# Project-MONAI/MONAI

Hardware: NVIDIA H100
Metric: voxels/sec sliding-window inference (higher is better)
Workload: dtype f16

## Files before the change

### monai_b200/_kernels.py

```python
from __future__ import annotations

import ctypes as C
import os
import weakref
from typing import Sequence

import torch

from . import _lib as L


class _Prof:
    on = False
    events: list = []


def profile_start() -> None:
    _Prof.on, _Prof.events = True, []


def profile_stop(by_shape: bool = False) -> dict:
    torch.cuda.synchronize()
    _Prof.on = False
    out: dict = {}
    for name, e0, e1, flops, nbytes in _Prof.events:
        if by_shape:
            name = f"{name} [{flops / 1e9:.2f} GF, {nbytes / 1e6:.1f} MB]"
        d = out.setdefault(name, {"ms": 0.0, "n": 0, "flops": 0.0, "bytes": 0.0})
        d["ms"] += e0.elapsed_time(e1)
        d["n"] += 1
        d["flops"] += flops
        d["bytes"] += nbytes
    _Prof.events = []
    return out


def _call(name: str, *args, flops: float = 0.0, nbytes: float = 0.0) -> None:
    fn = getattr(L.load(), "b200_" + name)
    dev = L.take_stream_device()
    if dev is not None and dev.index is not None and dev.index != torch.cuda.current_device():
        with torch.cuda.device(dev):
            return _call_on(fn, name, args, flops, nbytes)
    return _call_on(fn, name, args, flops, nbytes)


def _call_on(fn, name, args, flops, nbytes) -> None:
    if _Prof.on:
        e0, e1 = torch.cuda.Event(enable_timing=True), torch.cuda.Event(enable_timing=True)
        e0.record()
        rc = fn(*args)
        e1.record()
        _Prof.events.append((name, e0, e1, flops, nbytes))
    else:
        rc = fn(*args)
    L.check(rc, name)


_F32_CACHE: dict = {}


def _f32c(t: torch.Tensor | None) -> torch.Tensor | None:
    if t is None:
        return None
    src = t
    t = t.detach()
    if t.dtype == torch.float32 and t.is_contiguous():
        return t
    key = (id(src), tuple(t.shape), t.dtype, t.device)
    hit = _F32_CACHE.get(key)
    if hit is not None and hit[0]() is src and hit[1] == src._version and hit[2] == src.data_ptr():
        return hit[3]
    val = t.to(torch.float32).contiguous()
    try:
        ref = weakref.ref(src, lambda _r, k=key: _F32_CACHE.pop(k, None))
    except TypeError:
        return val
    _F32_CACHE[key] = (ref, src._version, src.data_ptr(), val)
    return val


def _ws(nbytes: int, device) -> torch.Tensor | None:
    if nbytes < 0:
        raise ValueError("monai_b200: workspace query failed for this shape")
    return torch.empty(max(int(nbytes), 16), device=device, dtype=torch.uint8)


# ... 548 lines not shown


def patch_merge_ln_nc8(x: NC8, gamma: torch.Tensor, beta: torch.Tensor, eps: float = 1e-5, v2: bool = False) -> NC8:
    sp2 = tuple((s + 1) // 2 for s in x.sp)
    out = NC8(x.N, 8 * x.C, sp2, x.buf.device)
    g, b = _f32c(gamma), _f32c(beta)
    _call("patch_merge_ln_nc8", L.ptr(x.buf), x.N, x.C, x.sp[0], x.sp[1], x.sp[2], L.ptr(g), L.ptr(b), float(eps), int(v2), L.ptr(out.buf), L.stream_ptr(x.buf.device))
    return out


def window_attention_nc8(qkv: NC8, Cc: int, heads: int, nW: int, n: int, scale: float, table: torch.Tensor, window: Sequence[int],
                         region: torch.Tensor | None) -> NC8:
    out = NC8(qkv.N, Cc, qkv.sp, qkv.buf.device)
    tab = _f32c(table)
    _call("window_attention_nc8", L.ptr(qkv.buf), qkv.N, Cc, heads, nW, n, float(scale), L.ptr(tab), int(window[0]), int(window[1]), int(window[2]),
          L.ptr(region), L.ptr(out.buf), L.stream_ptr(qkv.buf.device), flops=4.0 * qkv.N * nW * heads * n * n * 16,
          nbytes=float(qkv.N * 4 * Cc * nW * n * 2))
    return out


def window_attention_tc_plan(region, nW: int, n: int):
    import numpy as np

    if region is None:
        types = np.zeros(nW, dtype=np.int64)
        reps = None
        ntypes = 1
    else:
        region = np.asarray(region).reshape(nW, n)
        canon = np.empty_like(region)
        for w in range(nW):
            _, first, inv = np.unique(region[w], return_index=True, return_inverse=True)
            order = np.argsort(np.argsort(first))
            canon[w] = order[inv]
        uniq, types = np.unique(canon, axis=0, return_inverse=True)
        types = types.reshape(-1)
        ntypes = int(uniq.shape[0])
        reps = uniq.astype(np.int32)
    sched = np.zeros(16 + nW, dtype=np.int32)
    if ntypes <= 8:
        pos = 0
        for t in range(ntypes):
            ids = np.nonzero(types == t)[0]
            sched[t], sched[8 + t] = len(ids), pos
            sched[16 + pos: 16 + pos + len(ids)] = ids
            pos += len(ids)
    return sched, reps, ntypes


def window_attention_tc_pack_bias(table: torch.Tensor, heads: int, n: int, window: Sequence[int], region_types: torch.Tensor | None, ntypes: int) -> torch.Tensor:
    tab = _f32c(table)
    nbytes = L.load().b200_window_attention_tc_bias_bytes(heads, n, ntypes)
    if nbytes < 0:
        raise ValueError(f"window_attention_tc: unsupported shape (n={n}, mask types={ntypes})")
    packed = torch.empty(nbytes // 2, device=tab.device, dtype=torch.float16)
    _call("window_attention_tc_pack_bias", L.ptr(tab), heads, n, int(window[0]), int(window[1]), int(window[2]), L.ptr(region_types), ntypes,
          L.ptr(packed), L.stream_ptr(tab.device))
    return packed


def window_attention_tc(qkv: NC8, Cc: int, heads: int, nW: int, n: int, packed_bias: torch.Tensor, sched: torch.Tensor, ntypes: int) -> NC8:
    out = NC8(qkv.N, Cc, qkv.sp, qkv.buf.device)
    n_pad = (n + 31) // 32 * 32
    _call("window_attention_tc", L.ptr(qkv.buf), qkv.N, Cc, heads, nW, n, L.ptr(packed_bias), L.ptr(sched), ntypes, L.ptr(out.buf),
          L.stream_ptr(qkv.buf.device), flops=4.0 * qkv.N * nW * heads * n * n * 16, nbytes=float(qkv.N * 4 * Cc * nW * n * 2))
    return out


def mhsa_tc(qkv: NC8, C_: int, heads: int) -> NC8:
    if qkv.C != 3 * C_:
        raise ValueError(f"mhsa_tc: qkv has {qkv.C} channels, expected 3 * {C_}")
    out = NC8(qkv.N, C_, qkv.sp, qkv.buf.device)
    S = qkv.S
    try:
        _call("mhsa_tc", L.ptr(qkv.buf), qkv.N, C_, heads, S, L.ptr(out.buf), L.stream_ptr(qkv.buf.device),
              flops=4.0 * qkv.N * heads * S * S * 64, nbytes=float(qkv.N * 4 * C_ * S * 2))
    except RuntimeError as e:
        if C_ != 64 * heads:
            raise ValueError(str(e)) from None
        raise
    return out


ATTN_TC = not bool(os.environ.get("B200_ATTN_HMMA"))
LOG2E = 1.4426950408889634


def conv_cin1_nc8(x: torch.Tensor, weight: torch.Tensor, bias: torch.Tensor | None, k: int, stride: int, pad: int,
                  out: NC8 | None = None, out_coff: int = 0, want_stats: bool = False) -> tuple[NC8, torch.Tensor | None]:
    L.require_cuda(x)
    x = x.contiguous()
    N, _, D, H, W = x.shape
    Cout = weight.shape[0]
    sp = tuple((s + 2 * pad - k) // stride + 1 for s in (D, H, W))
    if out is None:
        out = NC8(N, Cout, sp, x.device)
    w32 = _f32c(weight)
    b32 = _f32c(bias)
    stats = torch.empty((N * Cout, 2), device=x.device, dtype=torch.float32) if want_stats else None
    tc = (k, stride, pad) in ((3, 1, 1), (2, 2, 0)) and Cout in (16, 32, 48, 64, 96, 128)
    name = "conv_cin1_tc" if tc else "conv_cin1_nc8"
    ws = None
    if want_stats:
        ws = _ws(getattr(L.load(), f"b200_{name}_workspace_bytes")(N, D, H, W, Cout, k, stride, pad), x.device)
    _call(name, L.ptr(x), L.dt(x), N, D, H, W, L.ptr(w32), L.ptr(b32), Cout, k, stride, pad, L.ptr(out.buf), out.C, out_coff, L.ptr(stats), L.ptr(ws),
          L.stream_ptr(x.device), flops=2.0 * N * sp[0] * sp[1] * sp[2] * Cout * k**3, nbytes=_nb(x) + float(N * sp[0] * sp[1] * sp[2] * Cout * 2))
    return out, stats


def head_conv_nc8(x: NC8, weight: torch.Tensor, bias: torch.Tensor | None, out_dtype: torch.dtype = torch.float16) -> torch.Tensor:
    Cout = weight.shape[0]
    w32 = _f32c(weight)
    b32 = _f32c(bias)
    y = torch.empty((x.N, Cout, *x.sp), device=x.buf.device, dtype=out_dtype)
    _call("head_conv_nc8", L.ptr(x.buf), x.N, x.C, x.S, L.ptr(w32), L.ptr(b32), Cout, L.ptr(y), L.dt(y), L.stream_ptr(x.buf.device))
    return y


def head_conv_norm_nc8(x: NC8, stats: torch.Tensor, res: NC8 | None, res_coff: int, res_stats: torch.Tensor | None, slope: float, eps: float,
                       weight: torch.Tensor, bias: torch.Tensor | None, out_dtype: torch.dtype = torch.float16) -> torch.Tensor:
    Cout = weight.shape[0]
    w32 = _f32c(weight)
    b32 = _f32c(bias)
    y = torch.empty((x.N, Cout, *x.sp), device=x.buf.device, dtype=out_dtype)
    _call("head_conv_norm_nc8", L.ptr(x.buf), x.N, x.C, x.S, L.ptr(stats), float(eps), L.ptr(res.buf) if res is not None else None,
          res.C if res is not None else 0, res_coff, L.ptr(res_stats), float(slope), L.ptr(w32), L.ptr(b32), Cout, L.ptr(y), L.dt(y),
          L.stream_ptr(x.buf.device), nbytes=float(x.N * x.S * (x.C * (4 if res is not None else 2) + Cout * y.element_size())))
    return y


def _cg_desc(x_sp, N, Cin, Cout, k, stride, pad, transposed, output_padding, in_ctot, in_coff, out_ctot, out_coff, out_layout, out_dtype):
    sp_out = conv_out_shape(x_sp, (k,) * 3, (stride,) * 3, (pad,) * 3, transposed, (output_padding,) * 3)
    return L.ConvGatherDesc(N, Cin, Cout, x_sp[0], x_sp[1], x_sp[2], sp_out[0], sp_out[1], sp_out[2], k, stride, pad, int(transposed),
                            in_ctot, in_coff, out_ctot, out_coff, out_layout, out_dtype), sp_out


def conv_gather_tc_pack_weight(weight: torch.Tensor, k: int, stride: int, pad: int, transposed: bool) -> torch.Tensor:
    L.require_cuda(weight)
    Cin, Cout = (weight.shape[0], weight.shape[1]) if transposed else (weight.shape[1], weight.shape[0])
    d, _ = _cg_desc((8, 8, 8), 1, Cin, Cout, k, stride, pad, transposed, stride - 1 if transposed else 0, Cin, 0, (Cout + 7) // 8 * 8, 0, 1, L.DT_F16)
    nbytes = L.load().b200_conv_gather_tc_weight_bytes(C.byref(d))
    if nbytes < 0:
        raise ValueError(f"conv_gather_tc needs Cin % 16 == 0, kernel <= 3, stride <= 2 (got Cin={Cin}, k={k}, stride={stride})")
    w32 = weight.detach().float().contiguous()
    packed = torch.empty(nbytes // 2, device=weight.device, dtype=torch.float16)
    _call("conv_gather_tc_pack_weight", C.byref(d), L.ptr(w32), L.ptr(packed), L.stream_ptr(weight.device))
    return packed


def conv_gather_tc(
    x: NC8, packed_w: torch.Tensor, Cin: int, Cout: int, k: int, stride: int, pad: int, transposed: bool = False, output_padding: int = 0,
    in_coff: int = 0, bias: torch.Tensor | None = None, out: "NC8 | torch.Tensor | None" = None, out_coff: int = 0,
    ncdhw_dtype: torch.dtype | None = None, want_stats: bool = False,
):
    layout = 0 if ncdhw_dtype is None else 1
    d, sp_out = _cg_desc(x.sp, x.N, Cin, Cout, k, stride, pad, transposed, output_padding, x.C, in_coff,
                         (out.C if isinstance(out, NC8) else (Cout + 7) // 8 * 8), out_coff, layout, L.dt(ncdhw_dtype) if layout else L.DT_F16)
    if out is None:
        out = NC8(x.N, Cout, sp_out, x.buf.device) if layout == 0 else torch.empty((x.N, Cout, *sp_out), device=x.buf.device, dtype=ncdhw_dtype)
        d.out_ctot = out.C if layout == 0 else d.out_ctot
    stats = torch.empty((x.N * Cout, 2), device=x.buf.device, dtype=torch.float32) if want_stats else None
    b32 = _f32c(bias)
    taps = k**3 if not transposed else (k**3) / (stride**3)
    ws = _ws(L.load().b200_conv_gather_tc_workspace_bytes(C.byref(d)), x.buf.device) if want_stats else None
    _call("conv_gather_tc", C.byref(d), L.ptr(x.buf), L.ptr(packed_w), L.ptr(b32), L.ptr(out.buf if layout == 0 else out), L.ptr(stats), L.ptr(ws),
          L.stream_ptr(x.buf.device), flops=2.0 * x.N * sp_out[0] * sp_out[1] * sp_out[2] * Cin * Cout * taps,
          nbytes=float(x.N * (x.S * Cin + sp_out[0] * sp_out[1] * sp_out[2] * Cout) * 2) + _nb(packed_w))
# ... 10 lines not shown
```

### monai_b200/csrc/attn_tc.cu

```cuda
#include "common.cuh"
#include "tc90.cuh"
#include "../../include/monai_b200.h"

namespace b200 {

constexpr int kAtNPadMax = 352;
constexpr int kAtKChunk = kAtNPadMax * 16;
constexpr int kAtBiasBytes = 16 * kAtNPadMax * 16;
constexpr int kAtIdBytes = 16 * 2048;
constexpr int kAtQBytes = 2 * 2048, kAtKBytes = 2 * kAtKChunk, kAtVBytes = 2 * kAtKChunk;
constexpr int kAtSmem = kAtBiasBytes + kAtIdBytes + 2 * (kAtQBytes + kAtKBytes + kAtVBytes) + 2 * 2 * tc::kStageFloats * 4 + 256 + 128;
constexpr float kAtPadBias = -30000.f;

struct AttnTcParams {
  const __half* qkv; __half* out; const __half* bias; const int32_t* sched;
  int N, C8, heads, nW, n, n_pad, nrt, ntypes;
};

struct AttnTile { int ty, h, rt, b, w; };

__device__ __forceinline__ AttnTile attn_decode(const AttnTcParams& p, long long f) {
  const int32_t* cnt = p.sched;
  const int32_t* start = p.sched + 8;
  const int32_t* win = p.sched + 16;
  AttnTile t;
  t.ty = 0;
  const long long hr_n = (long long)p.heads * p.nrt;
  for (;;) {
    const long long blk = (long long)cnt[t.ty] * p.N * hr_n;
    if (f < blk || t.ty + 1 >= p.ntypes) break;
    f -= blk; ++t.ty;
  }
  const int c = cnt[t.ty];
  const long long per = (long long)c * p.N;
  const int hr = (int)(f / per);
  const int l2 = (int)(f % per);
  t.h = hr / p.nrt; t.rt = hr % p.nrt;
  t.b = l2 / c;
  t.w = win[start[t.ty] + l2 % c];
  return t;
}

__device__ __forceinline__ float ex2(float x) {
  float y;
  asm("ex2.approx.ftz.f32 %0, %1;" : "=f"(y) : "f"(x));
  return y;
}

__device__ __forceinline__ uint32_t exp2_pack(float a, float b, float m, float& sum) {
  const __half2 h = __floats2half2_rn(ex2(a - m), ex2(b - m));
  const float2 r = __half22float2(h);
  sum += r.x + r.y;
  return *reinterpret_cast<const uint32_t*>(&h);
}

constexpr int kAtThreads = 384;

template <int NPAD>
__global__ void __launch_bounds__(kAtThreads, 1) window_attention_tc_kernel(AttnTcParams p) {
  extern __shared__ uint8_t smem_raw[];
  uint8_t* smem = tc::align_smem128(smem_raw);
  uint8_t* s_bias = smem;
  uint8_t* s_id = s_bias + kAtBiasBytes;
  uint8_t* s_q = s_id + kAtIdBytes;
  uint8_t* s_k = s_q + 2 * kAtQBytes;
  uint8_t* s_v = s_k + 2 * kAtKBytes;
  float* s_stage = reinterpret_cast<float*>(s_v + 2 * kAtVBytes);
  uint64_t* bars = reinterpret_cast<uint64_t*>(s_stage + 2 * 2 * tc::kStageFloats);
  uint64_t* qk_full = bars + 0;
  uint64_t* qk_empty = bars + 2;
  uint64_t* v_full = bars + 4;
  uint64_t* v_empty = bars + 6;

  const int warp = __shfl_sync(0xffffffffu, threadIdx.x >> 5, 0), lane = threadIdx.x & 31;
  constexpr int n_pad = NPAD;
  const int n = p.n;
  const long long T = (long long)p.nW * n;
  const long long total = (long long)p.N * p.nW * p.heads * p.nrt;
  const long long lo = total * blockIdx.x / gridDim.x, hi = total * (blockIdx.x + 1) / gridDim.x;

  if (threadIdx.x == 0) {
    for (int i = 0; i < 2; ++i) {
      tc::mbar_init(&qk_full[i], 1); tc::mbar_init(&qk_empty[i], 2); tc::mbar_init(&v_full[i], 1); tc::mbar_init(&v_empty[i], 2);
    }
    tc::fence_barrier_init();
  }
  {
    const uint4 z = make_uint4(0, 0, 0, 0);
    uint4* zq = reinterpret_cast<uint4*>(s_id);
    const int nz = (kAtIdBytes + 2 * kAtQBytes + 2 * kAtKBytes + 2 * kAtVBytes) / 16;
    for (int i = threadIdx.x; i < nz; i += blockDim.x) zq[i] = z;
  }
  __syncthreads();
  {
    __half* id = reinterpret_cast<__half*>(s_id);
    for (int r = threadIdx.x; r < 128; r += blockDim.x) id[((r >> 3) * 128 + r) * 8 + (r & 7)] = __float2half_rn(1.f);
  }
  tc::fence_proxy_async();
  __syncthreads();

  if (warp == 0) {
    if (lane == 0) {
      int last_combo = -1;
      int it = 0;
      for (long long f = lo; f < hi; ++f, ++it) {
        const AttnTile t = attn_decode(p, f);
        const int combo = (t.ty * p.heads + t.h) * p.nrt + t.rt;
        const int rows = min(128, n - t.rt * 128);
        const int b = it & 1;
        const uint32_t use = (uint32_t)((it >> 1) & 1);
        tc::mbar_wait(&qk_empty[b], use ^ 1u);
        uint32_t bias_bytes = 0u;
        if (combo != last_combo) {
          if (it > 0) tc::mbar_wait(&qk_empty[b ^ 1], (uint32_t)(((it - 1) >> 1) & 1));
          bias_bytes = (uint32_t)(16 * n_pad * 16);
        }
        tc::mbar_arrive_expect_tx(&qk_full[b], bias_bytes + 2u * rows * 16u + 2u * n * 16u);
        if (bias_bytes) tc::bulk_load(s_bias, p.bias + (long long)combo * (16 * n_pad * 8), bias_bytes, &qk_full[b]);
        last_combo = combo;
        const __half* base = p.qkv + (long long)t.b * (3 * p.C8) * T * 8;
        const long long row0 = (long long)t.w * n;
        for (int c = 0; c < 2; ++c) {
          tc::bulk_load(s_q + b * kAtQBytes + c * 2048, base + ((long long)(2 * t.h + c) * T + row0 + t.rt * 128) * 8, rows * 16, &qk_full[b]);
          tc::bulk_load(s_k + b * kAtKBytes + c * kAtKChunk, base + ((long long)(p.C8 + 2 * t.h + c) * T + row0) * 8, n * 16, &qk_full[b]);
        }
        tc::mbar_wait(&v_empty[b], use ^ 1u);
        tc::mbar_arrive_expect_tx(&v_full[b], 2u * n * 16u);
        for (int c = 0; c < 2; ++c)
          tc::bulk_load(s_v + b * kAtVBytes + c * kAtKChunk, base + ((long long)(2 * p.C8 + 2 * t.h + c) * T + row0) * 8, n * 16, &v_full[b]);
      }
    }
    __syncwarp();
  } else if (warp >= 4) {
    const int g = (warp >> 2) - 1, wid = warp & 3;
    const uint32_t q_a = tc::smem_u32(s_q), k_a = tc::smem_u32(s_k), v_a = tc::smem_u32(s_v), b_a = tc::smem_u32(s_bias),
                   i_a = tc::smem_u32(s_id);
    float* stage = s_stage + g * 2 * tc::kStageFloats;
    int sl = 0;
    int it = 0;
    for (long long f = lo; f < hi; ++f, ++it) {
      const int b = it & 1;
      const uint32_t use = (uint32_t)((it >> 1) & 1);
      float o[8];
#pragma unroll
      for (int j = 0; j < 8; ++j) o[j] = 0.f;
      float m0 = -INFINITY, m1 = -INFINITY, l0 = 0.f, l1 = 0.f;
      tc::mbar_wait(&qk_full[b], use);
      tc::mbar_wait(&v_full[b], use);
      const uint64_t qd = tc::make_desc_kmajor_noswz(q_a + b * kAtQBytes + g * 1024, 2048, 128);
#pragma unroll 1
      for (int kb = 0; kb < n_pad / 32; ++kb) {
        float sc[16];
        tc::wg_fence();
        tc::Mma<32>::ss<0>(sc, qd, tc::make_desc_kmajor_noswz(k_a + b * kAtKBytes + kb * 32 * 16, kAtKChunk, 128), 0u);
#pragma unroll
        for (int s4 = 0; s4 < 4; ++s4) {
          const int ks = 4 * g + s4;
          const uint64_t id_d = tc::make_desc_kmajor_noswz(i_a + ks * 4096 + g * 1024, 2048, 128);
          const uint64_t bd = tc::make_desc_kmajor_noswz(b_a + (2 * ks) * n_pad * 16 + kb * 32 * 16, n_pad * 16, 128);
          tc::Mma<32>::ss<0>(sc, id_d, bd, 1u);
        }
        tc::wg_commit();
        tc::wg_wait<0>();
        tc::wg_fence_acc<16>(sc);
        float x0 = sc[0], x1 = sc[2];
#pragma unroll
        for (int i = 0; i < 4; ++i) {
          x0 = fmaxf(x0, fmaxf(sc[4 * i], sc[4 * i + 1]));
          x1 = fmaxf(x1, fmaxf(sc[4 * i + 2], sc[4 * i + 3]));
        }
        x0 = fmaxf(x0, __shfl_xor_sync(0xffffffffu, x0, 1)); x0 = fmaxf(x0, __shfl_xor_sync(0xffffffffu, x0, 2));
        x1 = fmaxf(x1, __shfl_xor_sync(0xffffffffu, x1, 1)); x1 = fmaxf(x1, __shfl_xor_sync(0xffffffffu, x1, 2));
        const float n0 = fmaxf(m0, x0), n1 = fmaxf(m1, x1);
        const float a0 = ex2(m0 - n0), a1 = ex2(m1 - n1);
        m0 = n0; m1 = n1;
        l0 *= a0; l1 *= a1;
#pragma unroll
        for (int i = 0; i < 2; ++i) { o[4 * i] *= a0; o[4 * i + 1] *= a0; o[4 * i + 2] *= a1; o[4 * i + 3] *= a1; }
        uint32_t pa[2][4];
#pragma unroll
        for (int kk = 0; kk < 2; ++kk) {
          pa[kk][0] = exp2_pack(sc[8 * kk + 0], sc[8 * kk + 1], m0, l0);
          pa[kk][1] = exp2_pack(sc[8 * kk + 2], sc[8 * kk + 3], m1, l1);
          pa[kk][2] = exp2_pack(sc[8 * kk + 4], sc[8 * kk + 5], m0, l0);
          pa[kk][3] = exp2_pack(sc[8 * kk + 6], sc[8 * kk + 7], m1, l1);
        }
        tc::wg_fence();
#pragma unroll
        for (int kk = 0; kk < 2; ++kk) {
          const uint64_t vd = tc::make_desc_kmajor_noswz(v_a + b * kAtVBytes + (2 * kb + kk) * 256, 128, kAtKChunk);
          tc::Mma<16>::rs<1>(o, pa[kk], vd, 1u);
        }
        tc::wg_commit();
        tc::wg_wait<0>();
        tc::wg_fence_acc<8>(o);
#pragma unroll
        for (int kk = 0; kk < 2; ++kk)
#pragma unroll
          for (int j = 0; j < 4; ++j) asm volatile("" : "+r"(pa[kk][j])::"memory");
      }
      if (wid == 0 && lane == 0) { tc::mbar_arrive(&qk_empty[b]); tc::mbar_arrive(&v_empty[b]); }
      l0 += __shfl_xor_sync(0xffffffffu, l0, 1); l0 += __shfl_xor_sync(0xffffffffu, l0, 2);
      l1 += __shfl_xor_sync(0xffffffffu, l1, 1); l1 += __shfl_xor_sync(0xffffffffu, l1, 2);
      const float i0 = 1.f / l0, i1 = 1.f / l1;
#pragma unroll
      for (int i = 0; i < 2; ++i) { o[4 * i] *= i0; o[4 * i + 1] *= i0; o[4 * i + 2] *= i1; o[4 * i + 3] *= i1; }
      float* buf = stage + (sl & 1) * tc::kStageFloats;
      ++sl;
      tc::wg_stage16<0>(o, buf, wid, lane);
      tc::wg_bar(8 + g);
      float v[8];
      tc::wg_read8(buf, wid, lane, v);
      const AttnTile t = attn_decode(p, f);
      const int r = t.rt * 128 + 64 * g + 32 * (wid & 1) + lane;
      if (r < n) {
        const int dt = wid >> 1;
        __half* ob = p.out + (long long)t.b * p.C8 * T * 8 + ((long long)t.w * n + r) * 8;
        uint4 hv;
        __half2* hp = reinterpret_cast<__half2*>(&hv);
#pragma unroll
        for (int j = 0; j < 4; ++j) hp[j] = __floats2half2_rn(v[2 * j], v[2 * j + 1]);
        *reinterpret_cast<uint4*>(ob + (long long)(2 * t.h + dt) * T * 8) = hv;
      }
    }
  }
}

__global__ void attn_bias_pack_kernel(const float* __restrict__ table, const int32_t* __restrict__ region, __half* __restrict__ out,
                                      int heads, int n, int n_pad, int nrt, int ntypes, int ws0, int ws1, int ws2) {
  const long long total = (long long)ntypes * heads * nrt * 16 * n_pad * 8;
  const int s1 = 2 * ws2 - 1, s0 = (2 * ws1 - 1) * s1;
  const int lin_c = (ws0 - 1) * s0 + (ws1 - 1) * s1 + (ws2 - 1);
  constexpr float kLog2e = 1.4426950408889634f;
  for (long long i = (long long)blockIdx.x * blockDim.x + threadIdx.x; i < total; i += (long long)gridDim.x * blockDim.x) {
    long long r = i;
    const int e = (int)(r % 8); r /= 8;
    const int j = (int)(r % n_pad); r /= n_pad;
    const int c = (int)(r % 16); r /= 16;
    const int rt = (int)(r % nrt); r /= nrt;
    const int h = (int)(r % heads); r /= heads;
    const int ty = (int)r;
    const int ig = rt * 128 + c * 8 + e;
    float v;
    if (j >= n) v = kAtPadBias;
    else if (ig >= n) v = 0.f;
    else {
      const int li = (ig / (ws1 * ws2)) * s0 + ((ig / ws2) % ws1) * s1 + ig % ws2;
      const int lj = (j / (ws1 * ws2)) * s0 + ((j / ws2) % ws1) * s1 + j % ws2;
      v = table[(long long)(li - lj + lin_c) * heads + h] * kLog2e;
      if (region && region[(long long)ty * n + ig] != region[(long long)ty * n + j]) v += -100.f * kLog2e;
    }
    out[i] = __float2half_rn(v);
  }
}

}

using namespace b200;

static bool attn_tc_shape_ok(int heads, int n, int ntypes) {
  return heads > 0 && n > 0 && n <= kAtNPadMax && ntypes >= 1 && ntypes <= 8;
}

extern "C" long long b200_window_attention_tc_bias_bytes(int heads, int n, int ntypes) {
  if (!attn_tc_shape_ok(heads, n, ntypes) || n > kAtNPadMax) return -1;
  const int n_pad = (n + 31) / 32 * 32, nrt = (n + 127) / 128;
  return (long long)ntypes * heads * nrt * 16 * n_pad * 16;
}

extern "C" int b200_window_attention_tc_pack_bias(const float* table, int heads, int n, int ws0, int ws1, int ws2,
                                                  const int32_t* region_types, int ntypes, void* packed, void* stream) {
  B200_REQUIRE(table && packed, "window_attention_tc_pack_bias: null pointer");
  B200_REQUIRE(attn_tc_shape_ok(heads, n, ntypes) && n <= kAtNPadMax, "window_attention_tc: unsupported shape (n = %d, types = %d)", n, ntypes);
  B200_REQUIRE(ws0 > 0 && ws1 > 0 && ws2 > 0 && n <= ws0 * ws1 * ws2, "window_attention_tc: window of %d tokens exceeds the module window", n);
  B200_REQUIRE(ntypes == 1 || region_types, "window_attention_tc_pack_bias: several mask types need their region rows");
  const int n_pad = (n + 31) / 32 * 32, nrt = (n + 127) / 128;
  const long long total = (long long)ntypes * heads * nrt * 16 * n_pad * 8;
  const int blocks = (int)std::min<long long>((total + 255) / 256, 8192);
  attn_bias_pack_kernel<<<blocks, 256, 0, (cudaStream_t)stream>>>(table, region_types, (__half*)packed, heads, n, n_pad, nrt, ntypes, ws0, ws1, ws2);
  B200_LAUNCH_CHECK("attn_bias_pack_kernel");
  return B200_OK;
}

extern "C" int b200_window_attention_tc(const void* qkv, int N, int C, int heads, int nW, int n, const void* packed_bias,
                                        const int32_t* sched, int ntypes, void* out, void* stream) {
  B200_REQUIRE(qkv && out && packed_bias && sched, "window_attention_tc: null pointer");
  B200_REQUIRE(N > 0 && nW > 0, "window_attention_tc: empty problem");
  B200_REQUIRE(C == heads * 16, "window_attention_tc: head_dim must be 16 (C = %d, heads = %d)", C, heads);
  B200_REQUIRE(attn_tc_shape_ok(heads, n, ntypes) && n <= kAtNPadMax, "window_attention_tc: unsupported shape (n = %d, types = %d)", n, ntypes);
  AttnTcParams p;
  p.qkv = (const __half*)qkv; p.out = (__half*)out; p.bias = (const __half*)packed_bias; p.sched = sched;
  p.N = N; p.C8 = C / 8; p.heads = heads; p.nW = nW; p.n = n; p.n_pad = (n + 31) / 32 * 32; p.nrt = (n + 127) / 128; p.ntypes = ntypes;
  const long long total = (long long)N * nW * heads * p.nrt;
  dim3 grid((unsigned)std::min<long long>(total, num_sms()));
  void (*kern)(AttnTcParams) = nullptr;
  switch (p.n_pad) {
#define B200_ATTN_CASE(NP) case NP: kern = window_attention_tc_kernel<NP>; break;
    B200_ATTN_CASE(32) B200_ATTN_CASE(64) B200_ATTN_CASE(96) B200_ATTN_CASE(128) B200_ATTN_CASE(160) B200_ATTN_CASE(192)
    B200_ATTN_CASE(224) B200_ATTN_CASE(256) B200_ATTN_CASE(288) B200_ATTN_CASE(320) B200_ATTN_CASE(352)
#undef B200_ATTN_CASE
  }
  B200_REQUIRE(kern != nullptr, "window_attention_tc: no kernel for %d padded keys", p.n_pad);
  B200_CUDA(cudaFuncSetAttribute(kern, cudaFuncAttributeMaxDynamicSharedMemorySize, kAtSmem));
  kern<<<grid, kAtThreads, kAtSmem, (cudaStream_t)stream>>>(p);
  B200_LAUNCH_CHECK("window_attention_tc_kernel");
  return B200_OK;
}
```

### monai_b200/networks/nets/swin_unetr.py

```python
from __future__ import annotations

import itertools
from collections.abc import Sequence

import numpy as np
import torch
import torch.nn as nn

from ... import _kernels as K
from ... import _lib as L
from .._graph import GraphedForward
from ._tc_blocks import TcBlocks, _Cache
from ..blocks.acti_norm import norm_act_from_modules
from ..blocks.convolutions import Convolution, run_conv_module

__all__ = ["SwinUNETR", "PatchMerging", "PatchMergingV2", "window_plan"]


def _rep(v, n):
    return tuple(v) if isinstance(v, (list, tuple)) else (v,) * n


class PatchEmbed(nn.Module):

# ... 209 lines not shown
    ) -> None:
        super().__init__()
        if spatial_dims not in (2, 3):
            raise ValueError("spatial dimension should be 2 or 3.")
        for name, v in (("dropout rate", drop_rate), ("attention dropout rate", attn_drop_rate), ("drop path rate", dropout_path_rate)):
            if not (0 <= v <= 1):
                raise ValueError(f"{name} should be between 0 and 1.")
        if feature_size % 12 != 0:
            raise ValueError("feature_size should be divisible by 12.")
        if spatial_dims != 3:
            raise NotImplementedError("monai_b200 SwinUNETR implements spatial_dims=3")
        head_dims = [(feature_size * 2**i) // h for i, h in enumerate(num_heads)]
        if any((feature_size * 2**i) % h for i, h in enumerate(num_heads)) or any(d not in (8, 16, 24, 32, 48, 64) for d in head_dims):
            raise NotImplementedError(f"monai_b200 window attention supports head dimensions 8, 16, 24, 32, 48, 64 (got {head_dims})")
        self._tc_ok = feature_size % 48 == 0 and all(d == 16 for d in head_dims)
        self.fp32_faithful = False
        nn_name = norm_name if isinstance(norm_name, str) else norm_name[0]
        if str(nn_name).lower() != "instance" or (not isinstance(norm_name, str) and norm_name[1].get("affine")):
            raise NotImplementedError("monai_b200 SwinUNETR implements norm_name='instance' (non-affine)")
        if patch_size != 2:
            raise NotImplementedError("monai_b200 SwinUNETR implements patch_size=2")
        self.patch_size = patch_size
        self.normalize = normalize
        self.feature_size = feature_size
        self.out_channels = out_channels
        self.in_channels = in_channels
        if in_channels < 1:
            raise ValueError("in_channels must be positive")
        self.use_v2 = use_v2
        ws = _rep(window_size, 3)
        self.swinViT = SwinTransformer(in_channels, feature_size, ws, _rep(patch_size, 3), depths, num_heads, mlp_ratio, qkv_bias,
                                       norm_layer, patch_norm, downsample, use_v2)
        fs = feature_size
        self.encoder1 = UnetrBasicBlock(in_channels, fs)
        self.encoder2 = UnetrBasicBlock(fs, fs)
        self.encoder3 = UnetrBasicBlock(2 * fs, 2 * fs)
        self.encoder4 = UnetrBasicBlock(4 * fs, 4 * fs)
        self.encoder10 = UnetrBasicBlock(16 * fs, 16 * fs)
        self.decoder5 = UnetrUpBlock(16 * fs, 8 * fs)
        self.decoder4 = UnetrUpBlock(8 * fs, 4 * fs)
        self.decoder3 = UnetrUpBlock(4 * fs, 2 * fs)
        self.decoder2 = UnetrUpBlock(2 * fs, fs)
        self.decoder1 = UnetrUpBlock(fs, fs)
        self.out = UnetOutBlock(fs, out_channels)
        self._cache = _Cache()
        self._graph_init()

    def _check_input_size(self, spatial_shape):
        img_size = np.array(spatial_shape)
        remainder = (img_size % np.power(self.patch_size, 5)) > 0
        if remainder.any():
            wrong_dims = (np.where(remainder)[0] + 2).tolist()
            raise ValueError(
                f"spatial dimensions {wrong_dims} of input image (spatial shape: {spatial_shape})"
                f" must be divisible by {self.patch_size}**5."
            )

    def _plan(self, dims, ws, ss, dev):
        def build():
            src, region, nW, n = window_plan(dims, ws, ss)
            sched, reps, ntypes = K.window_attention_tc_plan(region, nW, n)
            tc = None
            if ntypes <= 8 and n <= 352:
                tc = (torch.from_numpy(sched).to(dev), None if reps is None else torch.from_numpy(reps).contiguous().to(dev), ntypes)
            return (torch.from_numpy(src).to(dev), None if region is None else torch.from_numpy(region).to(dev), nW, n, tc)

        return self._cache.get(("plan", tuple(dims), tuple(ws), tuple(ss), dev), [], build)

    def _attn_bias(self, attn: WindowAttention, key, n: int, tc):
        _, reps, ntypes = tc
        return self._cache.get(("attnb", key, n, ntypes, attn.relative_position_bias_table.device), [attn.relative_position_bias_table],
                               lambda: K.window_attention_tc_pack_bias(attn.relative_position_bias_table, attn.num_heads, n, attn.window_size, reps, ntypes))

    def _swin_stage(self, cur: K.NC8, layer: BasicLayer, key: str, pre: UnetrBasicBlock | None = None) -> K.NC8:
        dims, C = cur.sp, cur.C
        dev = cur.buf.device
        if pre is not None:
            cur = self._res_block(cur, C, 0, pre.layer, key + ".c")
        for bi, blk in enumerate(layer.blocks):
            ws, ss = _get_window_size(dims, blk.window_size, blk.shift_size)
            src, region, nW, n, tc = self._plan(dims, ws, ss, dev)
            bkey = f"{key}.b{bi}"
            xw = K.layernorm_nc8(cur, blk.norm1.weight, blk.norm1.bias, blk.norm1.eps, src=src, out_sp=(1, nW, n))
            if K.ATTN_TC and tc is not None:
                wq, bq = self._wqkv_scaled(blk.attn.qkv.weight, blk.attn.qkv.bias, C, blk.attn.scale, bkey)
                qkv, _ = K.gemm_tc(xw, wq, C, 3 * C, bias=bq)
                att = K.window_attention_tc(qkv, C, blk.num_heads, nW, n, self._attn_bias(blk.attn, (bkey, tuple(dims), tuple(ws), tuple(ss)), n, tc), tc[0], tc[2])
            else:
                qkv, _ = K.gemm_tc(xw, self._wlin(blk.attn.qkv.weight, bkey + ".qkv"), C, 3 * C, bias=blk.attn.qkv.bias)
                att = K.window_attention_nc8(qkv, C, blk.num_heads, nW, n, blk.attn.scale, blk.attn.relative_position_bias_table, blk.attn.window_size,
                                             region if any(s > 0 for s in ss) else None)
            x1, _ = K.gemm_tc(att, self._wlin(blk.attn.proj.weight, bkey + ".proj"), C, C, bias=blk.attn.proj.bias, res=cur, row_map=src, out_sp=dims, mode=1)
            hid = blk.mlp.linear1.out_features
            w1, w2 = self._wlin(blk.mlp.linear1.weight, bkey + ".fc1"), self._wlin(blk.mlp.linear2.weight, bkey + ".fc2")
            if K.mlp_fused_supported(C, hid):
                cur = K.mlp_fused_tc(x1, w1, blk.mlp.linear1.bias, w2, blk.mlp.linear2.bias, hid, blk.norm2.weight, blk.norm2.bias, blk.norm2.eps)
            else:
                y = K.layernorm_nc8(x1, blk.norm2.weight, blk.norm2.bias, blk.norm2.eps)
                h, _ = K.gemm_tc(y, w1, C, hid, bias=blk.mlp.linear1.bias, act=L.ACT_GELU)
                cur, _ = K.gemm_tc(h, w2, hid, C, bias=blk.mlp.linear2.bias, res=x1)
        if layer.downsample is not None:
            ds = layer.downsample
            m = K.patch_merge_ln_nc8(cur, ds.norm.weight, ds.norm.bias, ds.norm.eps, v2=ds.v2)
            cur, _ = K.gemm_tc(m, self._wlin(ds.reduction.weight, key + ".red"), 8 * C, 2 * C)
        return cur

    def _proj_out(self, t: K.NC8, out: K.NC8 | None = None, out_coff: int = 0) -> K.NC8:
        if not self.normalize:
            if out is None:
                return t
            return K.norm_act_nc8(t, t.C, None, out=out, out_coff=out_coff)
        if out is None:
            return K.layernorm_nc8(t, None, None, 1e-5)
        tmp = K.layernorm_nc8(t, None, None, 1e-5)
        return K.norm_act_nc8(tmp, t.C, None, out=out, out_coff=out_coff)

    def forward(self, x_in: torch.Tensor) -> torch.Tensor:
        if not x_in.is_cuda:
            raise RuntimeError("monai_b200.SwinUNETR runs on CUDA tensors only (there is no CPU fallback)")
        self._check_input_size(x_in.shape[2:])
        if x_in.shape[1] != self.in_channels:
            raise ValueError(f"expected {self.in_channels} input channel(s), got {x_in.shape[1]}")
        if x_in.dtype not in (torch.float16, torch.float32):
            raise TypeError(f"SwinUNETR takes float16/float32 inputs, got {x_in.dtype}")
        if not self._tc_ok or self.fp32_faithful:
            return self._forward_direct(x_in)
        if x_in.dtype == torch.float32 and not getattr(self, "_warned_fp32", False):
            import warnings

            warnings.warn("monai_b200.SwinUNETR computes with fp16 activation storage (fp32 accumulation); float32 inputs are converted. "
                          "Expect ~1e-2 relative agreement with an fp32 reference, not 1e-3 (set net.fp32_faithful = True for the fp32 path).")
            self._warned_fp32 = True
        if self._graph_ok():
            return self._forward_graphed(x_in, self._forward_impl)
        return self._forward_impl(x_in)

    def _plan_direct(self, dims, ws, ss, dev):
        key = ("plan_direct", tuple(dims), tuple(ws), tuple(ss), dev)
        hit = self._cache.store.get(key)
        if hit is None:
            src, region, nW, n = window_plan(dims, ws, ss)
            inv = np.full(int(np.prod(dims)), -1, dtype=np.int32)
            rows = np.nonzero(src >= 0)[0]
            inv[src[rows]] = rows.astype(np.int32)
            hit = (torch.from_numpy(src).to(dev), None if region is None else torch.from_numpy(np.ascontiguousarray(region)).to(dev),
                   torch.from_numpy(inv).to(dev), nW, n)
            self._cache.store[key] = hit
        return hit

    def _dense_bias(self, attn: WindowAttention, n: int, key):
        def build():
            idx = attn.relative_position_index[:n, :n].reshape(-1)
            return attn.relative_position_bias_table.detach().float()[idx].reshape(n, n, -1).permute(2, 0, 1).contiguous()

        return self._cache.get(("dense_bias", key, n, attn.relative_position_bias_table.device), [attn.relative_position_bias_table], build)

    def _merge_params(self, ds, C: int, key):
        def build():
            order = list(itertools.product(range(2), range(2), range(2))) if ds.v2 else \
                [(0, 0, 0), (1, 0, 0), (0, 1, 0), (0, 0, 1), (1, 1, 0), (1, 0, 1), (0, 1, 1), (1, 1, 1)]
            ref_of_pat = np.empty(8 * C, dtype=np.int64)
            for k, (a, b, e) in enumerate(order):
                for c in range(C):
                    ref_of_pat[c * 8 + a * 4 + b * 2 + e] = k * C + c
            idx = torch.from_numpy(ref_of_pat).to(ds.norm.weight.device)
            return (ds.norm.weight.detach().float()[idx].contiguous(), ds.norm.bias.detach().float()[idx].contiguous(),
                    ds.reduction.weight.detach().float()[:, idx].contiguous())
# ... 149 lines not shown
```

Measured before the change: 55.56 million.

## Restructure window attention kernel: three consumer warpgroups, bias preloaded into accumulators, pipelined QK/PV

Rewrites the tensor-core window attention kernel to use three consumer warpgroups covering 192 query rows, up from two covering 128. The relative position bias is now repacked into accumulator-fragment layout and loaded straight into the score registers, replacing the extra identity-matrix MMAs that added it before. The QK^T MMA for the next 64-key chunk is issued while softmax and the PV MMA of the current chunk run. Register budgets are rebalanced with setmaxnreg, and the schedule groups tiles so bias reloads happen less often. The trade-offs are higher register pressure and more complex synchronisation, and the environment switch that selected the older fallback path is removed.

```diff
diff --git a/monai_b200/_kernels.py b/monai_b200/_kernels.py
--- a/monai_b200/_kernels.py
+++ b/monai_b200/_kernels.py
@@ -1,7 +1,6 @@
 from __future__ import annotations
 
 import ctypes as C
-import os
 import weakref
 from typing import Sequence
 
@@ -716,7 +715,6 @@
     return out
 
 
-ATTN_TC = not bool(os.environ.get("B200_ATTN_HMMA"))
 LOG2E = 1.4426950408889634
 
 
diff --git a/monai_b200/csrc/attn_tc.cu b/monai_b200/csrc/attn_tc.cu
--- a/monai_b200/csrc/attn_tc.cu
+++ b/monai_b200/csrc/attn_tc.cu
@@ -5,12 +5,15 @@
 namespace b200 {
 
 constexpr int kAtNPadMax = 352;
+constexpr int kAtWG = 3;
+constexpr int kAtRows = 64 * kAtWG;
+constexpr int kAtCT = 128 * kAtWG;
 constexpr int kAtKChunk = kAtNPadMax * 16;
-constexpr int kAtBiasBytes = 16 * kAtNPadMax * 16;
-constexpr int kAtIdBytes = 16 * 2048;
-constexpr int kAtQBytes = 2 * 2048, kAtKBytes = 2 * kAtKChunk, kAtVBytes = 2 * kAtKChunk;
-constexpr int kAtSmem = kAtBiasBytes + kAtIdBytes + 2 * (kAtQBytes + kAtKBytes + kAtVBytes) + 2 * 2 * tc::kStageFloats * 4 + 256 + 128;
+constexpr int kAtBiasBytes = kAtNPadMax * kAtCT;
+constexpr int kAtQBytes = 2 * kAtRows * 16, kAtKBytes = 2 * kAtKChunk, kAtVBytes = 2 * kAtKChunk;
+constexpr int kAtSmem = kAtBiasBytes + 2 * (kAtQBytes + kAtKBytes + kAtVBytes) + kAtWG * 2 * tc::kStageFloats * 4 + 256 + 128;
 constexpr float kAtPadBias = -30000.f;
+constexpr int kAtGroup = 8;
 
 struct AttnTcParams {
   const __half* qkv; __half* out; const __half* bias; const int32_t* sched;
@@ -32,10 +35,23 @@
     f -= blk; ++t.ty;
   }
   const int c = cnt[t.ty];
-  const long long per = (long long)c * p.N;
-  const int hr = (int)(f / per);
-  const int l2 = (int)(f % per);
-  t.h = hr / p.nrt; t.rt = hr % p.nrt;
+  const int per = c * p.N;
+  const long long per_h = (long long)per * p.nrt;
+  t.h = (int)(f / per_h);
+  int r = (int)(f % per_h);
+  const int full = per / kAtGroup * kAtGroup;
+  int l2;
+  if (r < full * p.nrt) {
+    const int grp = r / (kAtGroup * p.nrt);
+    r %= kAtGroup * p.nrt;
+    t.rt = r / kAtGroup;
+    l2 = grp * kAtGroup + r % kAtGroup;
+  } else {
+    r -= full * p.nrt;
+    const int rem = per - full;
+    t.rt = r / rem;
+    l2 = full + r % rem;
+  }
   t.b = l2 / c;
   t.w = win[start[t.ty] + l2 % c];
   return t;
@@ -54,19 +70,28 @@
   return *reinterpret_cast<const uint32_t*>(&h);
 }
 
-constexpr int kAtThreads = 384;
+__device__ __forceinline__ void bias_to_acc(const uint8_t* src, float* d) {
+  const uint4 v = *reinterpret_cast<const uint4*>(src);
+  const __half2* h = reinterpret_cast<const __half2*>(&v);
+#pragma unroll
+  for (int j = 0; j < 4; ++j) {
+    const float2 f = __half22float2(h[j]);
+    d[2 * j] = f.x; d[2 * j + 1] = f.y;
+  }
+}
+
+constexpr int kAtThreads = 128 * (kAtWG + 1);
 
 template <int NPAD>
 __global__ void __launch_bounds__(kAtThreads, 1) window_attention_tc_kernel(AttnTcParams p) {
   extern __shared__ uint8_t smem_raw[];
   uint8_t* smem = tc::align_smem128(smem_raw);
   uint8_t* s_bias = smem;
-  uint8_t* s_id = s_bias + kAtBiasBytes;
-  uint8_t* s_q = s_id + kAtIdBytes;
+  uint8_t* s_q = s_bias + kAtBiasBytes;
   uint8_t* s_k = s_q + 2 * kAtQBytes;
   uint8_t* s_v = s_k + 2 * kAtKBytes;
   float* s_stage = reinterpret_cast<float*>(s_v + 2 * kAtVBytes);
-  uint64_t* bars = reinterpret_cast<uint64_t*>(s_stage + 2 * 2 * tc::kStageFloats);
+  uint64_t* bars = reinterpret_cast<uint64_t*>(s_stage + kAtWG * 2 * tc::kStageFloats);
   uint64_t* qk_full = bars + 0;
   uint64_t* qk_empty = bars + 2;
   uint64_t* v_full = bars + 4;
@@ -74,6 +99,8 @@
 
   const int warp = __shfl_sync(0xffffffffu, threadIdx.x >> 5, 0), lane = threadIdx.x & 31;
   constexpr int n_pad = NPAD;
+  constexpr int NB = NPAD / 32;
+  constexpr int NC = (NB + 1) / 2;
   const int n = p.n;
   const long long T = (long long)p.nW * n;
   const long long total = (long long)p.N * p.nW * p.heads * p.nrt;
@@ -81,47 +108,43 @@
 
   if (threadIdx.x == 0) {
     for (int i = 0; i < 2; ++i) {
-      tc::mbar_init(&qk_full[i], 1); tc::mbar_init(&qk_empty[i], 2); tc::mbar_init(&v_full[i], 1); tc::mbar_init(&v_empty[i], 2);
+      tc::mbar_init(&qk_full[i], 1); tc::mbar_init(&qk_empty[i], kAtWG); tc::mbar_init(&v_full[i], 1); tc::mbar_init(&v_empty[i], kAtWG);
     }
     tc::fence_barrier_init();
   }
   {
     const uint4 z = make_uint4(0, 0, 0, 0);
-    uint4* zq = reinterpret_cast<uint4*>(s_id);
-    const int nz = (kAtIdBytes + 2 * kAtQBytes + 2 * kAtKBytes + 2 * kAtVBytes) / 16;
+    uint4* zq = reinterpret_cast<uint4*>(s_q);
+    const int nz = (2 * kAtQBytes + 2 * kAtKBytes + 2 * kAtVBytes) / 16;
     for (int i = threadIdx.x; i < nz; i += blockDim.x) zq[i] = z;
-  }
-  __syncthreads();
-  {
-    __half* id = reinterpret_cast<__half*>(s_id);
-    for (int r = threadIdx.x; r < 128; r += blockDim.x) id[((r >> 3) * 128 + r) * 8 + (r & 7)] = __float2half_rn(1.f);
   }
   tc::fence_proxy_async();
   __syncthreads();
 
-  if (warp == 0) {
-    if (lane == 0) {
+  if (warp < 4) {
+    asm volatile("setmaxnreg.dec.sync.aligned.u32 56;\n" ::: "memory");
+    if (warp == 0 && lane == 0) {
       int last_combo = -1;
       int it = 0;
       for (long long f = lo; f < hi; ++f, ++it) {
         const AttnTile t = attn_decode(p, f);
         const int combo = (t.ty * p.heads + t.h) * p.nrt + t.rt;
-        const int rows = min(128, n - t.rt * 128);
+        const int rows = min(kAtRows, n - t.rt * kAtRows);
         const int b = it & 1;
         const uint32_t use = (uint32_t)((it >> 1) & 1);
         tc::mbar_wait(&qk_empty[b], use ^ 1u);
         uint32_t bias_bytes = 0u;
         if (combo != last_combo) {
           if (it > 0) tc::mbar_wait(&qk_empty[b ^ 1], (uint32_t)(((it - 1) >> 1) & 1));
-          bias_bytes = (uint32_t)(16 * n_pad * 16);
+          bias_bytes = (uint32_t)(n_pad * kAtCT);
         }
         tc::mbar_arrive_expect_tx(&qk_full[b], bias_bytes + 2u * rows * 16u + 2u * n * 16u);
-        if (bias_bytes) tc::bulk_load(s_bias, p.bias + (long long)combo * (16 * n_pad * 8), bias_bytes, &qk_full[b]);
+        if (bias_bytes) tc::bulk_load(s_bias, p.bias + (long long)combo * (n_pad * kAtCT / 2), bias_bytes, &qk_full[b]);
         last_combo = combo;
         const __half* base = p.qkv + (long long)t.b * (3 * p.C8) * T * 8;
         const long long row0 = (long long)t.w * n;
         for (int c = 0; c < 2; ++c) {
-          tc::bulk_load(s_q + b * kAtQBytes + c * 2048, base + ((long long)(2 * t.h + c) * T + row0 + t.rt * 128) * 8, rows * 16, &qk_full[b]);
+          tc::bulk_load(s_q + b * kAtQBytes + c * kAtRows * 16, base + ((long long)(2 * t.h + c) * T + row0 + t.rt * kAtRows) * 8, rows * 16, &qk_full[b]);
           tc::bulk_load(s_k + b * kAtKBytes + c * kAtKChunk, base + ((long long)(p.C8 + 2 * t.h + c) * T + row0) * 8, n * 16, &qk_full[b]);
         }
         tc::mbar_wait(&v_empty[b], use ^ 1u);
@@ -130,79 +153,116 @@
           tc::bulk_load(s_v + b * kAtVBytes + c * kAtKChunk, base + ((long long)(2 * p.C8 + 2 * t.h + c) * T + row0) * 8, n * 16, &v_full[b]);
       }
     }
-    __syncwarp();
-  } else if (warp >= 4) {
+  } else {
+    asm volatile("setmaxnreg.inc.sync.aligned.u32 152;\n" ::: "memory");
     const int g = (warp >> 2) - 1, wid = warp & 3;
-    const uint32_t q_a = tc::smem_u32(s_q), k_a = tc::smem_u32(s_k), v_a = tc::smem_u32(s_v), b_a = tc::smem_u32(s_bias),
-                   i_a = tc::smem_u32(s_id);
+    const int ct = threadIdx.x - 128;
+    const uint32_t q_a = tc::smem_u32(s_q), k_a = tc::smem_u32(s_k), v_a = tc::smem_u32(s_v);
     float* stage = s_stage + g * 2 * tc::kStageFloats;
     int sl = 0;
     int it = 0;
     for (long long f = lo; f < hi; ++f, ++it) {
       const int b = it & 1;
       const uint32_t use = (uint32_t)((it >> 1) & 1);
+      const AttnTile t = attn_decode(p, f);
+      const bool dead = t.rt * kAtRows + 64 * g + 16 * wid >= n;
       float o[8];
 #pragma unroll
       for (int j = 0; j < 8; ++j) o[j] = 0.f;
       float m0 = -INFINITY, m1 = -INFINITY, l0 = 0.f, l1 = 0.f;
+      float s[2][32];
+      uint32_t pa[2][4][4];
       tc::mbar_wait(&qk_full[b], use);
       tc::mbar_wait(&v_full[b], use);
-      const uint64_t qd = tc::make_desc_kmajor_noswz(q_a + b * kAtQBytes + g * 1024, 2048, 128);
-#pragma unroll 1
-      for (int kb = 0; kb < n_pad / 32; ++kb) {
-        float sc[16];
+      if (t.rt * kAtRows + 64 * g >= n) {
+        if (wid == 0 && lane == 0) { tc::mbar_arrive(&qk_empty[b]); tc::mbar_arrive(&v_empty[b]); }
+        continue;
+      }
+      const uint64_t qd = tc::make_desc_kmajor_noswz(q_a + b * kAtQBytes + g * 1024, kAtRows * 16, 128);
+
+      auto issue_s = [&](auto cc) {
+        constexpr int c = decltype(cc)::value;
+        constexpr int nb = (2 * c + 1 < NB) ? 2 : 1;
+        float* sc = s[c & 1];
+#pragma unroll
+        for (int k2 = 0; k2 < nb; ++k2)
+#pragma unroll
+          for (int hh = 0; hh < 2; ++hh) bias_to_acc(s_bias + ((2 * c + k2) * 2 + hh) * (kAtCT * 16) + ct * 16, sc + 16 * k2 + 8 * hh);
         tc::wg_fence();
-        tc::Mma<32>::ss<0>(sc, qd, tc::make_desc_kmajor_noswz(k_a + b * kAtKBytes + kb * 32 * 16, kAtKChunk, 128), 0u);
-#pragma unroll
-        for (int s4 = 0; s4 < 4; ++s4) {
-          const int ks = 4 * g + s4;
-          const uint64_t id_d = tc::make_desc_kmajor_noswz(i_a + ks * 4096 + g * 1024, 2048, 128);
-          const uint64_t bd = tc::make_desc_kmajor_noswz(b_a + (2 * ks) * n_pad * 16 + kb * 32 * 16, n_pad * 16, 128);
-          tc::Mma<32>::ss<0>(sc, id_d, bd, 1u);
-        }
+        const uint64_t kd = tc::make_desc_kmajor_noswz(k_a + b * kAtKBytes + c * 64 * 16, kAtKChunk, 128);
+        if constexpr (nb == 2) tc::Mma<64>::ss<0>(sc, qd, kd, 1u);
+        else tc::Mma<32>::ss<0>(sc, qd, kd, 1u);
         tc::wg_commit();
-        tc::wg_wait<0>();
-        tc::wg_fence_acc<16>(sc);
-        float x0 = sc[0], x1 = sc[2];
-#pragma unroll
-        for (int i = 0; i < 4; ++i) {
-          x0 = fmaxf(x0, fmaxf(sc[4 * i], sc[4 * i + 1]));
-          x1 = fmaxf(x1, fmaxf(sc[4 * i + 2], sc[4 * i + 3]));
-        }
-        x0 = fmaxf(x0, __shfl_xor_sync(0xffffffffu, x0, 1)); x0 = fmaxf(x0, __shfl_xor_sync(0xffffffffu, x0, 2));
-        x1 = fmaxf(x1, __shfl_xor_sync(0xffffffffu, x1, 1)); x1 = fmaxf(x1, __shfl_xor_sync(0xffffffffu, x1, 2));
-        const float n0 = fmaxf(m0, x0), n1 = fmaxf(m1, x1);
-        const float a0 = ex2(m0 - n0), a1 = ex2(m1 - n1);
-        m0 = n0; m1 = n1;
-        l0 *= a0; l1 *= a1;
+      };
+
+      issue_s(std::integral_constant<int, 0>{});
+      tc::static_for<0, NC>([&](auto cc) {
+        constexpr int c = decltype(cc)::value;
+        constexpr int nb = (2 * c + 1 < NB) ? 2 : 1;
+        constexpr int nv = 16 * nb;
+        if constexpr (c + 1 < NC) {
+          issue_s(std::integral_constant<int, c + 1>{});
+          if constexpr (c == 0) tc::wg_wait<1>(); else tc::wg_wait<2>();
+        } else {
+          if constexpr (c == 0) tc::wg_wait<0>(); else tc::wg_wait<1>();
+        }
+        float* sc = s[c & 1];
+        tc::wg_fence_acc<nv>(sc);
+        float a0 = 1.f, a1 = 1.f, ps0 = 0.f, ps1 = 0.f;
+        if (!dead) {
+          float x0 = sc[0], x1 = sc[2];
+#pragma unroll
+          for (int i = 0; i < nv / 4; ++i) {
+            x0 = fmaxf(x0, fmaxf(sc[4 * i], sc[4 * i + 1]));
+            x1 = fmaxf(x1, fmaxf(sc[4 * i + 2], sc[4 * i + 3]));
+          }
+          x0 = fmaxf(x0, __shfl_xor_sync(0xffffffffu, x0, 1)); x0 = fmaxf(x0, __shfl_xor_sync(0xffffffffu, x0, 2));
+          x1 = fmaxf(x1, __shfl_xor_sync(0xffffffffu, x1, 1)); x1 = fmaxf(x1, __shfl_xor_sync(0xffffffffu, x1, 2));
+          const float n0 = fmaxf(m0, x0), n1 = fmaxf(m1, x1);
+          a0 = ex2(m0 - n0); a1 = ex2(m1 - n1);
+          m0 = n0; m1 = n1;
+#pragma unroll
+          for (int kk = 0; kk < 2 * nb; ++kk) {
+            pa[c & 1][kk][0] = exp2_pack(sc[8 * kk + 0], sc[8 * kk + 1], m0, ps0);
+            pa[c & 1][kk][1] = exp2_pack(sc[8 * kk + 2], sc[8 * kk + 3], m1, ps1);
+            pa[c & 1][kk][2] = exp2_pack(sc[8 * kk + 4], sc[8 * kk + 5], m0, ps0);
+            pa[c & 1][kk][3] = exp2_pack(sc[8 * kk + 6], sc[8 * kk + 7], m1, ps1);
+          }
+        } else {
+#pragma unroll
+          for (int kk = 0; kk < 2 * nb; ++kk)
+#pragma unroll
+            for (int j = 0; j < 4; ++j) pa[c & 1][kk][j] = 0u;
+        }
+        if constexpr (c > 0) {
+          if constexpr (c + 1 < NC) tc::wg_wait<1>(); else tc::wg_wait<0>();
+          tc::wg_fence_acc<8>(o);
+#pragma unroll
+          for (int kk = 0; kk < 4; ++kk)
+#pragma unroll
+            for (int j = 0; j < 4; ++j) asm volatile("" : "+r"(pa[(c - 1) & 1][kk][j])::"memory");
+        }
+        l0 = l0 * a0 + ps0; l1 = l1 * a1 + ps1;
 #pragma unroll
         for (int i = 0; i < 2; ++i) { o[4 * i] *= a0; o[4 * i + 1] *= a0; o[4 * i + 2] *= a1; o[4 * i + 3] *= a1; }
-        uint32_t pa[2][4];
-#pragma unroll
-        for (int kk = 0; kk < 2; ++kk) {
-          pa[kk][0] = exp2_pack(sc[8 * kk + 0], sc[8 * kk + 1], m0, l0);
-          pa[kk][1] = exp2_pack(sc[8 * kk + 2], sc[8 * kk + 3], m1, l1);
-          pa[kk][2] = exp2_pack(sc[8 * kk + 4], sc[8 * kk + 5], m0, l0);
-          pa[kk][3] = exp2_pack(sc[8 * kk + 6], sc[8 * kk + 7], m1, l1);
-        }
         tc::wg_fence();
 #pragma unroll
-        for (int kk = 0; kk < 2; ++kk) {
-          const uint64_t vd = tc::make_desc_kmajor_noswz(v_a + b * kAtVBytes + (2 * kb + kk) * 256, 128, kAtKChunk);
-          tc::Mma<16>::rs<1>(o, pa[kk], vd, 1u);
+        for (int kk = 0; kk < 2 * nb; ++kk) {
+          const uint64_t vd = tc::make_desc_kmajor_noswz(v_a + b * kAtVBytes + (4 * c + kk) * 256, 128, kAtKChunk);
+          tc::Mma<16>::rs<1>(o, pa[c & 1][kk], vd, 1u);
         }
         tc::wg_commit();
-        tc::wg_wait<0>();
-        tc::wg_fence_acc<8>(o);
-#pragma unroll
-        for (int kk = 0; kk < 2; ++kk)
-#pragma unroll
-          for (int j = 0; j < 4; ++j) asm volatile("" : "+r"(pa[kk][j])::"memory");
-      }
+      });
+      tc::wg_wait<0>();
+      tc::wg_fence_acc<8>(o);
+#pragma unroll
+      for (int kk = 0; kk < 4; ++kk)
+#pragma unroll
+        for (int j = 0; j < 4; ++j) asm volatile("" : "+r"(pa[(NC - 1) & 1][kk][j])::"memory");
       if (wid == 0 && lane == 0) { tc::mbar_arrive(&qk_empty[b]); tc::mbar_arrive(&v_empty[b]); }
       l0 += __shfl_xor_sync(0xffffffffu, l0, 1); l0 += __shfl_xor_sync(0xffffffffu, l0, 2);
       l1 += __shfl_xor_sync(0xffffffffu, l1, 1); l1 += __shfl_xor_sync(0xffffffffu, l1, 2);
-      const float i0 = 1.f / l0, i1 = 1.f / l1;
+      const float i0 = dead ? 0.f : 1.f / l0, i1 = dead ? 0.f : 1.f / l1;
 #pragma unroll
       for (int i = 0; i < 2; ++i) { o[4 * i] *= i0; o[4 * i + 1] *= i0; o[4 * i + 2] *= i1; o[4 * i + 3] *= i1; }
       float* buf = stage + (sl & 1) * tc::kStageFloats;
@@ -211,8 +271,7 @@
       tc::wg_bar(8 + g);
       float v[8];
       tc::wg_read8(buf, wid, lane, v);
-      const AttnTile t = attn_decode(p, f);
-      const int r = t.rt * 128 + 64 * g + 32 * (wid & 1) + lane;
+      const int r = t.rt * kAtRows + 64 * g + 32 * (wid & 1) + lane;
       if (r < n) {
         const int dt = wid >> 1;
         __half* ob = p.out + (long long)t.b * p.C8 * T * 8 + ((long long)t.w * n + r) * 8;
@@ -228,19 +287,23 @@
 
 __global__ void attn_bias_pack_kernel(const float* __restrict__ table, const int32_t* __restrict__ region, __half* __restrict__ out,
                                       int heads, int n, int n_pad, int nrt, int ntypes, int ws0, int ws1, int ws2) {
-  const long long total = (long long)ntypes * heads * nrt * 16 * n_pad * 8;
+  const long long total = (long long)ntypes * heads * nrt * n_pad * (kAtCT / 2);
   const int s1 = 2 * ws2 - 1, s0 = (2 * ws1 - 1) * s1;
   const int lin_c = (ws0 - 1) * s0 + (ws1 - 1) * s1 + (ws2 - 1);
+  const int nb = n_pad / 32;
   constexpr float kLog2e = 1.4426950408889634f;
   for (long long i = (long long)blockIdx.x * blockDim.x + threadIdx.x; i < total; i += (long long)gridDim.x * blockDim.x) {
     long long r = i;
-    const int e = (int)(r % 8); r /= 8;
-    const int j = (int)(r % n_pad); r /= n_pad;
-    const int c = (int)(r % 16); r /= 16;
+    const int e8 = (int)(r % 8); r /= 8;
+    const int ct = (int)(r % kAtCT); r /= kAtCT;
+    const int hh = (int)(r % 2); r /= 2;
+    const int kb = (int)(r % nb); r /= nb;
     const int rt = (int)(r % nrt); r /= nrt;
     const int h = (int)(r % heads); r /= heads;
     const int ty = (int)r;
-    const int ig = rt * 128 + c * 8 + e;
+    const int v16 = 8 * hh + e8, cb = v16 >> 2, e = v16 & 3, l = ct & 31;
+    const int ig = rt * kAtRows + (ct >> 7) * 64 + ((ct >> 5) & 3) * 16 + (l >> 2) + (e >= 2 ? 8 : 0);
+    const int j = kb * 32 + cb * 8 + 2 * (l & 3) + (e & 1);
     float v;
     if (j >= n) v = kAtPadBias;
     else if (ig >= n) v = 0.f;
@@ -264,8 +327,8 @@
 
 extern "C" long long b200_window_attention_tc_bias_bytes(int heads, int n, int ntypes) {
   if (!attn_tc_shape_ok(heads, n, ntypes) || n > kAtNPadMax) return -1;
-  const int n_pad = (n + 31) / 32 * 32, nrt = (n + 127) / 128;
-  return (long long)ntypes * heads * nrt * 16 * n_pad * 16;
+  const int n_pad = (n + 31) / 32 * 32, nrt = (n + kAtRows - 1) / kAtRows;
+  return (long long)ntypes * heads * nrt * n_pad * kAtCT;
 }
 
 extern "C" int b200_window_attention_tc_pack_bias(const float* table, int heads, int n, int ws0, int ws1, int ws2,
@@ -274,8 +337,8 @@
   B200_REQUIRE(attn_tc_shape_ok(heads, n, ntypes) && n <= kAtNPadMax, "window_attention_tc: unsupported shape (n = %d, types = %d)", n, ntypes);
   B200_REQUIRE(ws0 > 0 && ws1 > 0 && ws2 > 0 && n <= ws0 * ws1 * ws2, "window_attention_tc: window of %d tokens exceeds the module window", n);
   B200_REQUIRE(ntypes == 1 || region_types, "window_attention_tc_pack_bias: several mask types need their region rows");
-  const int n_pad = (n + 31) / 32 * 32, nrt = (n + 127) / 128;
-  const long long total = (long long)ntypes * heads * nrt * 16 * n_pad * 8;
+  const int n_pad = (n + 31) / 32 * 32, nrt = (n + kAtRows - 1) / kAtRows;
+  const long long total = (long long)ntypes * heads * nrt * n_pad * (kAtCT / 2);
   const int blocks = (int)std::min<long long>((total + 255) / 256, 8192);
   attn_bias_pack_kernel<<<blocks, 256, 0, (cudaStream_t)stream>>>(table, region_types, (__half*)packed, heads, n, n_pad, nrt, ntypes, ws0, ws1, ws2);
   B200_LAUNCH_CHECK("attn_bias_pack_kernel");
@@ -290,7 +353,7 @@
   B200_REQUIRE(attn_tc_shape_ok(heads, n, ntypes) && n <= kAtNPadMax, "window_attention_tc: unsupported shape (n = %d, types = %d)", n, ntypes);
   AttnTcParams p;
   p.qkv = (const __half*)qkv; p.out = (__half*)out; p.bias = (const __half*)packed_bias; p.sched = sched;
-  p.N = N; p.C8 = C / 8; p.heads = heads; p.nW = nW; p.n = n; p.n_pad = (n + 31) / 32 * 32; p.nrt = (n + 127) / 128; p.ntypes = ntypes;
+  p.N = N; p.C8 = C / 8; p.heads = heads; p.nW = nW; p.n = n; p.n_pad = (n + 31) / 32 * 32; p.nrt = (n + kAtRows - 1) / kAtRows; p.ntypes = ntypes;
   const long long total = (long long)N * nW * heads * p.nrt;
   dim3 grid((unsigned)std::min<long long>(total, num_sms()));
   void (*kern)(AttnTcParams) = nullptr;
diff --git a/monai_b200/networks/nets/swin_unetr.py b/monai_b200/networks/nets/swin_unetr.py
--- a/monai_b200/networks/nets/swin_unetr.py
+++ b/monai_b200/networks/nets/swin_unetr.py
@@ -315,7 +315,7 @@
             src, region, nW, n, tc = self._plan(dims, ws, ss, dev)
             bkey = f"{key}.b{bi}"
             xw = K.layernorm_nc8(cur, blk.norm1.weight, blk.norm1.bias, blk.norm1.eps, src=src, out_sp=(1, nW, n))
-            if K.ATTN_TC and tc is not None:
+            if tc is not None:
                 wq, bq = self._wqkv_scaled(blk.attn.qkv.weight, blk.attn.qkv.bias, C, blk.attn.scale, bkey)
                 qkv, _ = K.gemm_tc(xw, wq, C, 3 * C, bias=bq)
                 att = K.window_attention_tc(qkv, C, blk.num_heads, nW, n, self._attn_bias(blk.attn, (bkey, tuple(dims), tuple(ws), tuple(ss)), n, tc), tc[0], tc[2])
```

Measured after the change: 59.17 million (median of 6 runs). 1.06x the previous value.
